# AnjieCheng/SpatialRGPT

Measured on NVIDIA H100. Metric: generated_tokens_per_sec, higher is better.
Workload: dtype bf16

## Files before the change

include/srgpt_b200.h:

```cpp
#ifndef SRGPT_B200_H_
#define SRGPT_B200_H_

#ifdef __cplusplus
extern "C" {
#endif

#define SRGPT_ABI_VERSION 1

int srgpt_abi_version(void);
int srgpt_elem_type(void);
const char* srgpt_last_error(void);
int srgpt_device_info(int* sm_count, int* cc_major, int* cc_minor);

int srgpt_trace_begin(void* device_buf, int capacity_records);
int srgpt_trace_end(void);

enum {
  SRGPT_EPI_NONE = 0,
  SRGPT_EPI_BIAS = 1,
  SRGPT_EPI_BIAS_GELU_TANH = 2,
  SRGPT_EPI_BIAS_GELU_ERF = 3,
  SRGPT_EPI_BIAS_RESIDUAL = 4,
  SRGPT_EPI_SWIGLU = 5,
  SRGPT_EPI_BIAS_QUICK_GELU = 6
};
long long srgpt_gemm_workspace_bytes(void);
int srgpt_gemm_set_workspace(void* workspace, long long bytes);
int srgpt_gemm_bf16(const void* A, int lda, const void* W, int ldw, void* C, int ldc, int M, int N, int K,
                    const void* bias , const void* residual , int ldr,
                    int res_row_mod , int epilogue, int out_fp32, void* stream);

int srgpt_layernorm_bf16(const void* x, int ldx, const void* weight, const void* bias, void* y, int ldy, int rows,
                         int cols, float eps, int act, void* stream);
int srgpt_downsample_layernorm_bf16(const void* x, const void* weight, const void* bias, void* y, int n_img, int side,
                                    int C, float eps, void* stream);
int srgpt_rmsnorm_bf16(const void* x, int ldx, const void* weight, void* y, int ldy, int rows, int cols, float eps,
                       void* stream);
int srgpt_patchify_bf16(const void* images, int src_is_bf16, void* A, int n, int R, int ps, int ldk, void* stream);
int srgpt_clip_embed_bf16(const void* patch_embeds, const void* class_embedding, const void* position_embedding, void* out,
                          int n_img, int T, int D, void* stream);
int srgpt_splice_rows_bf16(const void* src0, const void* src1, const void* src2, const void* src3, const int* src_id,
                           const int* src_row, void* out, int rows, int cols, void* stream);

long long srgpt_mask_weights_workspace(int n_img, int M, int side);
int srgpt_mask_weights(const void* masks, int mask_is_bf16, void* w, void* workspace, int n_img, int M, int IH, int IW,
                       int side, float rscale, int order, void* stream);
long long srgpt_mask_pool_workspace(int n_img, int M, int L, int C);
int srgpt_mask_pool_bf16(const void* x, const void* w, void* out, void* workspace, int n_img, int M, int L, int C,
                         void* stream);
int srgpt_adaptive_avgpool_bf16(const void* x, void* y, int n_img, int side, int out_side, int C, int order,
                                void* stream);
int srgpt_reorder_rows_bf16(const void* x, void* y, int n_img, int side, int C, int from_order, int to_order,
                            void* stream);
int srgpt_depth_to_u8x3(const void* depth, int h, int w, void* out, int H, int W, void* workspace, void* stream);

int srgpt_attention_prefill_bf16(const void* q, const void* k, const void* v, void* out, int q_ld, int kv_ld, int o_ld,
                                 int batch, int seqlen, int n_heads, int n_kv_heads, int head_dim, float scale,
                                 int causal, void* stream);
int srgpt_attention_prefill_varlen_bf16(const void* q, const void* k, const void* v, void* out, int q_ld, int kv_ld,
                                        int o_ld, int n_seqs, const int* cu_seqlens, int max_seqlen, int total_rows,
                                        int n_heads, int n_kv_heads, int head_dim, float scale, int causal, void* stream);
int srgpt_rope_kv_append_bf16(void* qkv, int rows, int n_heads, int n_kv_heads, int head_dim, const void* cos_tab,
                              const void* sin_tab, const int* start_pos, void* kv_pages, const int* page_table,
                              int page_size, void* stream);
int srgpt_rope_kv_append_varlen_bf16(void* qkv, int rows, int n_heads, int n_kv_heads, int head_dim, const void* cos_tab,
                                     const void* sin_tab, const int* start_pos, void* kv_pages, const int* page_tables,
                                     int page_table_stride, int page_size, int n_seqs, const int* cu_seqlens, void* stream);
int srgpt_attention_prefill_paged_bf16(const void* q, int q_ld, void* out, int o_ld, const void* kv_pages, int n_pages,
                                       const int* page_tables, int page_table_stride, int page_size, const int* start_pos,
                                       const int* cu_seqlens, int n_seqs, int max_rows, int total_rows, int n_heads, int n_kv_heads,
                                       int head_dim, float scale, void* stream);
int srgpt_rows_equal(const void* a, const void* b, int rows, long long row_bytes, int* flags, void* stream);
int srgpt_attention_decode_bf16(const void* q, void* out, const void* kv_pages, const int* page_table, int page_size,
                                const int* kv_len_minus1, int n_heads, int n_kv_heads, int head_dim, float scale,
                                void* stream);

enum { SRGPT_GEMV_PLAIN = 0, SRGPT_GEMV_SWIGLU = 1, SRGPT_GEMV_QKV_ROPE = 2 };
int srgpt_gemv_bf16(const void* x, const void* W, int ldw, void* y, int N, int K, const void* norm_weight, float eps,
                    const void* residual, int mode,
                     int n_heads, int n_kv_heads, int head_dim, const void* cos_tab,
                    const void* sin_tab, const int* pos, void* kv_pages, const int* page_table, int page_size,
                    void* stream);
long long srgpt_lm_head_workspace(int V);
// ... 273 lines not shown
```

spatialrgpt_b200/_lib.py:

```python
from __future__ import annotations

import ctypes as C
import os
import threading

from . import _build

_lock = threading.Lock()
_libs = {}
_elem = "bf16"


class SrgptError(RuntimeError):
    pass


vp, ci, cf, cll = C.c_void_p, C.c_int, C.c_float, C.c_longlong

SIGNATURES = {
    "srgpt_abi_version": (ci, []),
    "srgpt_elem_type": (ci, []),
    "srgpt_last_error": (C.c_char_p, []),
    "srgpt_device_info": (ci, [C.POINTER(ci), C.POINTER(ci), C.POINTER(ci)]),
    "srgpt_trace_begin": (ci, [vp, ci]),
    "srgpt_trace_end": (ci, []),
    "srgpt_gemm_workspace_bytes": (cll, []),
    "srgpt_gemm_set_workspace": (ci, [vp, cll]),
    "srgpt_gemm_bf16": (ci, [vp, ci, vp, ci, vp, ci, ci, ci, ci, vp, vp, ci, ci, ci, ci, vp]),
    "srgpt_layernorm_bf16": (ci, [vp, ci, vp, vp, vp, ci, ci, ci, cf, ci, vp]),
    "srgpt_downsample_layernorm_bf16": (ci, [vp, vp, vp, vp, ci, ci, ci, cf, vp]),
    "srgpt_rmsnorm_bf16": (ci, [vp, ci, vp, vp, ci, ci, ci, cf, vp]),
    "srgpt_patchify_bf16": (ci, [vp, ci, vp, ci, ci, ci, ci, vp]),
    "srgpt_clip_embed_bf16": (ci, [vp, vp, vp, vp, ci, ci, ci, vp]),
    "srgpt_splice_rows_bf16": (ci, [vp, vp, vp, vp, vp, vp, vp, ci, ci, vp]),
    "srgpt_mask_weights_workspace": (cll, [ci, ci, ci]),
    "srgpt_mask_weights": (ci, [vp, ci, vp, vp, ci, ci, ci, ci, ci, cf, ci, vp]),
    "srgpt_mask_pool_workspace": (cll, [ci, ci, ci, ci]),
    "srgpt_mask_pool_bf16": (ci, [vp, vp, vp, vp, ci, ci, ci, ci, vp]),
    "srgpt_adaptive_avgpool_bf16": (ci, [vp, vp, ci, ci, ci, ci, ci, vp]),
    "srgpt_reorder_rows_bf16": (ci, [vp, vp, ci, ci, ci, ci, ci, vp]),
    "srgpt_depth_to_u8x3": (ci, [vp, ci, ci, vp, ci, ci, vp, vp]),
    "srgpt_attention_prefill_bf16": (ci, [vp, vp, vp, vp, ci, ci, ci, ci, ci, ci, ci, ci, cf, ci, vp]),
    "srgpt_attention_prefill_varlen_bf16": (ci, [vp, vp, vp, vp, ci, ci, ci, ci, vp, ci, ci, ci, ci, ci, cf, ci, vp]),
    "srgpt_rope_kv_append_bf16": (ci, [vp, ci, ci, ci, ci, vp, vp, vp, vp, vp, ci, vp]),
    "srgpt_rope_kv_append_varlen_bf16": (ci, [vp, ci, ci, ci, ci, vp, vp, vp, vp, vp, ci, ci, ci, vp, vp]),
    "srgpt_attention_prefill_paged_bf16": (ci, [vp, ci, vp, ci, vp, ci, vp, ci, ci, vp, vp, ci, ci, ci, ci, ci, ci, cf, vp]),
    "srgpt_rows_equal": (ci, [vp, vp, ci, cll, vp, vp]),
    "srgpt_attention_decode_bf16": (ci, [vp, vp, vp, vp, ci, vp, ci, ci, ci, cf, vp]),
    "srgpt_gemv_bf16": (ci, [vp, vp, ci, vp, ci, ci, vp, cf, vp, ci, ci, ci, ci, vp, vp, vp, vp, vp, ci, vp]),
    "srgpt_lm_head_workspace": (cll, [ci]),
    "srgpt_lm_head_argmax_bf16": (ci, [vp, vp, ci, ci, ci, vp, cf, vp, vp, vp, vp, vp, vp, vp, vp]),
    "srgpt_argmax_f32": (ci, [vp, ci, ci, vp, vp]),
    "srgpt_argmax_bf16": (ci, [vp, ci, ci, ci, vp, vp]),
    "srgpt_beam_candidates_bf16": (ci, [vp, ci, ci, ci, vp, ci, vp, vp, vp]),
    "srgpt_beam_candidates_scores_bf16": (ci, [vp, ci, ci, ci, vp, ci, vp, vp, vp, cll, vp]),
    "srgpt_step_scores": (ci, [vp, ci, cll, ci, ci, vp, ci, vp, cll, cll, vp]),
    "srgpt_beam_select": (ci, [vp, vp, ci, ci, ci, vp, vp, vp, vp]),
    "srgpt_kv_copy_workspace_bytes": (cll, [ci, ci, ci, ci]),
    "srgpt_kv_copy_pages": (ci, [vp, ci, ci, ci, ci, vp, ci, ci, vp, cll, vp]),
    "srgpt_token_logprobs": (ci, [vp, cll, ci, ci, vp, vp, ci, vp, cll, vp, vp, vp, vp]),
    "srgpt_sample_top_p_f32": (ci, [vp, ci, vp, vp, vp, ci, vp, vp, vp, ci, vp]),
    "srgpt_sample_rows": (ci, [vp, ci, ci, ci, ci, vp, vp, vp, ci, vp, vp]),
    "srgpt_sample_top_p_scores_f32": (ci, [vp, ci, vp, vp, vp, ci, vp, vp, vp, ci, vp, cll, vp]),
    "srgpt_sample_rows_scores": (ci, [vp, ci, ci, ci, ci, vp, vp, vp, ci, vp, vp, cll, vp]),
    "srgpt_logits_process": (ci, [vp, ci, ci, ci, ci, vp, ci, ci, ci, vp, ci, vp, vp, ci, vp, ci, vp, vp]),
    "srgpt_logits_pick_token": (ci, [vp, vp, ci, vp, vp, vp, ci, vp]),
    "srgpt_resample_u8": (ci, [vp, vp, ci, ci, ci, ci, ci, vp, vp, ci, vp]),
    "srgpt_u8_to_normalized_chw": (ci, [vp, vp, ci, ci, ci, C.c_double, vp, vp, ci, vp]),
    "srgpt_resize_nearest_u8": (ci, [vp, vp, ci, ci, ci, ci, vp, vp, vp]),
    "srgpt_attention_decode_batched_bf16": (ci, [vp, ci, vp, ci, vp, vp, ci, ci, vp, ci, ci, ci, ci, cf, vp]),
    "srgpt_decode_batch_advance": (ci, [vp, vp, vp, ci, vp, vp, vp, ci, vp, vp]),
    "srgpt_gemv_tp_bf16": (ci, [vp, vp, ci, vp, ci, ci, vp, cf, ci, ci, ci, ci, vp, vp, vp, vp, vp, ci, ci, ci, vp, vp]),
    "srgpt_attention_decode_tp_bf16": (ci, [vp, vp, vp, vp, ci, vp, ci, ci, ci, ci, ci, cf, vp]),
    "srgpt_tp_residual_add_bf16": (ci, [vp, vp, ci, vp]),
    "srgpt_lm_head_local_best_bf16": (ci, [vp, vp, ci, ci, ci, vp, cf, vp, ci, vp, vp]),
    "srgpt_tp_pick_token": (ci, [vp, ci, vp, vp, ci, vp, vp, vp, vp]),
    "srgpt_tp_comm_bytes": (cll, [ci, ci, ci]),
    "srgpt_tp_comm_slot_offset": (cll, [ci, ci, ci]),
    "srgpt_tp_allreduce_residual_bf16": (ci, [vp, ci, ci, cll, ci, vp, vp, vp, ci, vp]),
    "srgpt_tp_allgather_pick_token": (ci, [vp, ci, ci, cll, ci, vp, vp, vp, ci, vp, vp, vp, vp]),
    "srgpt_siglip_layers_bf16": (ci, [vp, vp, ci, vp, vp, vp, vp, ci, ci, ci, ci, ci, cf, vp]),
# ... 169 lines not shown
```

spatialrgpt_b200/csrc/gemm_wgmma.cu:

```cuda
#include <cuda.h>
#include <stdlib.h>

#include "common.cuh"
#include "nf4.cuh"
#include "srgpt_b200.h"
#include "tma.cuh"

namespace srgpt {
namespace gemm {

using namespace tma;

constexpr int BM = 128, BN = 128, BK = 64;
constexpr int WG_K = 16;
constexpr int STAGES = 6;
constexpr int A_BYTES = BM * BK * 2;
constexpr int B_BYTES = BN * BK * 2;
constexpr int STAGE_BYTES = A_BYTES + B_BYTES;
constexpr int NUM_THREADS = 3 * 128;
constexpr int SMEM_BYTES = STAGES * STAGE_BYTES + 1024  + 256 ;
constexpr int TSK_MAX_CTAS = 256;
constexpr int TSK_FLAG_BYTES = TSK_MAX_CTAS * 4;
constexpr long long TSK_SLOT_FLOATS = (long long)BM * BN;

__device__ __forceinline__ unsigned int ld_acquire_u32(const unsigned int* p) {
  unsigned int v;
  asm volatile("ld.acquire.gpu.global.u32 %0, [%1];" : "=r"(v) : "l"(p) : "memory");
  return v;
}
__device__ __forceinline__ void st_release_u32(unsigned int* p, unsigned int v) {
  asm volatile("st.release.gpu.global.u32 [%0], %1;" ::"l"(p), "r"(v) : "memory");
}

__device__ __forceinline__ void wgmma_m64n128k16(float (&d)[64], uint64_t desc_a, uint64_t desc_b) {
  asm volatile(
      "{\n\t.reg .pred p;\n\tsetp.ne.b32 p, 1, 0;\n\t"
      "wgmma.mma_async.sync.aligned.m64n128k16.f32." SRGPT_ELEM_PTX "." SRGPT_ELEM_PTX " "
      "{%0, %1, %2, %3, %4, %5, %6, %7, %8, %9, %10, %11, %12, %13, %14, %15, "
      "%16, %17, %18, %19, %20, %21, %22, %23, %24, %25, %26, %27, %28, %29, %30, %31, "
      "%32, %33, %34, %35, %36, %37, %38, %39, %40, %41, %42, %43, %44, %45, %46, %47, "
      "%48, %49, %50, %51, %52, %53, %54, %55, %56, %57, %58, %59, %60, %61, %62, %63}, "
      "%64, %65, p, 1, 1, 0, 0;\n\t}"
      : "+f"(d[0]), "+f"(d[1]), "+f"(d[2]), "+f"(d[3]), "+f"(d[4]), "+f"(d[5]), "+f"(d[6]), "+f"(d[7]),
        "+f"(d[8]), "+f"(d[9]), "+f"(d[10]), "+f"(d[11]), "+f"(d[12]), "+f"(d[13]), "+f"(d[14]), "+f"(d[15]),
        "+f"(d[16]), "+f"(d[17]), "+f"(d[18]), "+f"(d[19]), "+f"(d[20]), "+f"(d[21]), "+f"(d[22]), "+f"(d[23]),
        "+f"(d[24]), "+f"(d[25]), "+f"(d[26]), "+f"(d[27]), "+f"(d[28]), "+f"(d[29]), "+f"(d[30]), "+f"(d[31]),
        "+f"(d[32]), "+f"(d[33]), "+f"(d[34]), "+f"(d[35]), "+f"(d[36]), "+f"(d[37]), "+f"(d[38]), "+f"(d[39]),
        "+f"(d[40]), "+f"(d[41]), "+f"(d[42]), "+f"(d[43]), "+f"(d[44]), "+f"(d[45]), "+f"(d[46]), "+f"(d[47]),
        "+f"(d[48]), "+f"(d[49]), "+f"(d[50]), "+f"(d[51]), "+f"(d[52]), "+f"(d[53]), "+f"(d[54]), "+f"(d[55]),
        "+f"(d[56]), "+f"(d[57]), "+f"(d[58]), "+f"(d[59]), "+f"(d[60]), "+f"(d[61]), "+f"(d[62]), "+f"(d[63])
      : "l"(desc_a), "l"(desc_b)
      : "memory");
}

__device__ __forceinline__ void wgmma_m64n128k32_e4m3(float (&d)[64], uint64_t desc_a, uint64_t desc_b) {
  asm volatile(
      "{\n\t.reg .pred p;\n\tsetp.ne.b32 p, 1, 0;\n\t"
      "wgmma.mma_async.sync.aligned.m64n128k32.f32.e4m3.e4m3 "
      "{%0, %1, %2, %3, %4, %5, %6, %7, %8, %9, %10, %11, %12, %13, %14, %15, "
      "%16, %17, %18, %19, %20, %21, %22, %23, %24, %25, %26, %27, %28, %29, %30, %31, "
      "%32, %33, %34, %35, %36, %37, %38, %39, %40, %41, %42, %43, %44, %45, %46, %47, "
      "%48, %49, %50, %51, %52, %53, %54, %55, %56, %57, %58, %59, %60, %61, %62, %63}, "
      "%64, %65, p, 1, 1;\n\t}"
      : "+f"(d[0]), "+f"(d[1]), "+f"(d[2]), "+f"(d[3]), "+f"(d[4]), "+f"(d[5]), "+f"(d[6]), "+f"(d[7]),
        "+f"(d[8]), "+f"(d[9]), "+f"(d[10]), "+f"(d[11]), "+f"(d[12]), "+f"(d[13]), "+f"(d[14]), "+f"(d[15]),
        "+f"(d[16]), "+f"(d[17]), "+f"(d[18]), "+f"(d[19]), "+f"(d[20]), "+f"(d[21]), "+f"(d[22]), "+f"(d[23]),
        "+f"(d[24]), "+f"(d[25]), "+f"(d[26]), "+f"(d[27]), "+f"(d[28]), "+f"(d[29]), "+f"(d[30]), "+f"(d[31]),
        "+f"(d[32]), "+f"(d[33]), "+f"(d[34]), "+f"(d[35]), "+f"(d[36]), "+f"(d[37]), "+f"(d[38]), "+f"(d[39]),
        "+f"(d[40]), "+f"(d[41]), "+f"(d[42]), "+f"(d[43]), "+f"(d[44]), "+f"(d[45]), "+f"(d[46]), "+f"(d[47]),
        "+f"(d[48]), "+f"(d[49]), "+f"(d[50]), "+f"(d[51]), "+f"(d[52]), "+f"(d[53]), "+f"(d[54]), "+f"(d[55]),
        "+f"(d[56]), "+f"(d[57]), "+f"(d[58]), "+f"(d[59]), "+f"(d[60]), "+f"(d[61]), "+f"(d[62]), "+f"(d[63])
      : "l"(desc_a), "l"(desc_b)
      : "memory");
}

struct Fp8Scales {
  const float* sx;
  const float* sw;
};

struct Params {
  int M, N, K;
  int ldc;
  const bf16* bias;
  const bf16* residual;
  int ldr;
  int res_row_mod;
  void* C;
  int out_fp32;
  int gm;
};

struct TskWs {
  float* partial;
  unsigned int* flags;
  unsigned int epoch;
};

__device__ __forceinline__ void unit_to_tile(int unit, int tiles_m, int tiles_n, int gm, int& mt, int& nt) {
  const int per_group = gm * tiles_n;
  const int g = unit / per_group;
  const int rem = unit - g * per_group;
  const int g0 = g * gm;
  const int gsz = min(gm, tiles_m - g0);
  nt = rem / gsz;
  mt = g0 + rem - nt * gsz;
}

template <int EPI>
__device__ __forceinline__ void store_acc(const float (&d)[64], const Params& p, int row0, int col0) {
#pragma unroll
  for (int i = 0; i < 2; ++i) {
    const int row = row0 + 8 * i;
    if (row >= p.M) continue;
    const int rrow = p.res_row_mod > 0 ? row % p.res_row_mod : row;
#pragma unroll
    for (int j = 0; j < 16; ++j) {
      const int col = col0 + 8 * j;
      if (col >= p.N) continue;
      const bool two = col + 1 < p.N;
      float v0 = d[4 * j + 2 * i], v1 = d[4 * j + 2 * i + 1];
      if (EPI == SRGPT_EPI_SWIGLU) {
        const float g = bf16_round(v0), u = bf16_round(v1);
        reinterpret_cast<bf16*>(p.C)[(size_t)row * p.ldc + (col >> 1)] = f2e(bf16_round(silu(g)) * u);
        continue;
      }
      if (EPI != SRGPT_EPI_NONE && p.bias != nullptr) {
        if (two) {
          const uint32_t b = *reinterpret_cast<const uint32_t*>(p.bias + col);
          v0 += bf16_lo(b);
          v1 += bf16_hi(b);
        } else {
          v0 += e2f(p.bias[col]);
        }
      }
      if (EPI == SRGPT_EPI_BIAS_GELU_TANH) {
        v0 = gelu_tanh(bf16_round(v0)); v1 = gelu_tanh(bf16_round(v1));
      } else if (EPI == SRGPT_EPI_BIAS_GELU_ERF) {
        v0 = gelu_erf(bf16_round(v0)); v1 = gelu_erf(bf16_round(v1));
      } else if (EPI == SRGPT_EPI_BIAS_QUICK_GELU) {
        v0 = quick_gelu(bf16_round(v0)); v1 = quick_gelu(bf16_round(v1));
      } else if (EPI == SRGPT_EPI_BIAS_RESIDUAL && p.residual != nullptr) {
        const bf16* rp = p.residual + (size_t)rrow * p.ldr + col;
        if (two) {
          const uint32_t r = *reinterpret_cast<const uint32_t*>(rp);
          v0 = bf16_round(v0) + bf16_lo(r);
          v1 = bf16_round(v1) + bf16_hi(r);
        } else {
          v0 = bf16_round(v0) + e2f(rp[0]);
        }
      }
      if (p.out_fp32) {
        float* cp = reinterpret_cast<float*>(p.C) + (size_t)row * p.ldc + col;
        if (two && (p.ldc & 1) == 0) {
          *reinterpret_cast<float2*>(cp) = make_float2(v0, v1);
        } else {
          cp[0] = v0;
          if (two) cp[1] = v1;
        }
      } else {
        bf16* cp = reinterpret_cast<bf16*>(p.C) + (size_t)row * p.ldc + col;
        if (two) {
          *reinterpret_cast<uint32_t*>(cp) = pack_bf16x2(v0, v1);
        } else {
          cp[0] = f2e(v0);
        }
      }
    }
  }
}
// ... 4 lines not shown
    const int row = row0 + 8 * i;
    if (row >= p.M) continue;
    const float sx = sc.sx[row];
#pragma unroll
    for (int j = 0; j < 16; ++j) {
      const int col = col0 + 8 * j;
#pragma unroll
      for (int c = 0; c < 2; ++c)
        if (col + c < p.N) d[4 * j + 2 * i + c] *= sx * sc.sw[col + c];
    }
  }
}

__device__ __forceinline__ void fence_proxy_async_shared() { asm volatile("fence.proxy.async.shared::cta;" ::: "memory"); }

struct Nf4Raw {
  uint32_t w[8];
  float s[8];
};

__device__ __forceinline__ void nf4_coords(bool sk, int i, int u_begin, int num_kb, int cta, int G, int tiles_m, int tiles_n, int gm, int& m0,
                                           int& n0, int& kb) {
  if (sk) {
    const int u = u_begin + i, tile = u / num_kb;
    m0 = 0;
    n0 = tile * BN;
    kb = u - tile * num_kb;
  } else {
    const int ui = i / num_kb;
    int mt, nt;
    unit_to_tile(cta + ui * G, tiles_m, tiles_n, gm, mt, nt);
    m0 = mt * BM;
    n0 = nt * BN;
    kb = i - ui * num_kb;
  }
}

__device__ __forceinline__ void nf4_fetch(const srgpt_nf4& w4, const Params& p, int n0, int kb, int r0, int j, Nf4Raw& c) {
  const size_t row_bytes = (size_t)(p.K >> 1);
  const int row_scales = p.K / nf4::BLOCK;
  const uint8_t* q = w4.q + (size_t)(n0 + r0) * row_bytes + nf4::lane_offset(8 * kb + j);
  const float* s = w4.scale + (size_t)(n0 + r0) * row_scales + kb;
#pragma unroll
  for (int i = 0; i < 8; ++i) {
    c.w[i] = 0x77777777u;
    c.s[i] = 0.f;
    if (n0 + r0 + 16 * i < p.N) {
      c.w[i] = __ldg(reinterpret_cast<const uint32_t*>(q + (size_t)(16 * i) * row_bytes));
      c.s[i] = __ldg(s + (size_t)(16 * i) * row_scales);
    }
  }
}

template <int EPI, bool SK, bool FP8, bool NF4 = false>
__device__ __forceinline__ void gemm_body(const CUtensorMap* tmap_a, const CUtensorMap* tmap_b, const Params& p, const TskWs& ws, const Fp8Scales& sc,
                                          const srgpt_nf4& w4 = srgpt_nf4{nullptr, nullptr}) {
  constexpr int KB = FP8 ? 128 : BK;
  extern __shared__ uint8_t smem_raw[];
  uint8_t* smem = reinterpret_cast<uint8_t*>((reinterpret_cast<uintptr_t>(smem_raw) + 1023) & ~(uintptr_t)1023);
  uint64_t* full_bar = reinterpret_cast<uint64_t*>(smem + STAGES * STAGE_BYTES);
  uint64_t* empty_bar = full_bar + STAGES;

  const int tiles_m = (p.M + BM - 1) / BM;
  const int tiles_n = (p.N + BN - 1) / BN;
  const int num_kb = (p.K + KB - 1) / KB;
  const int num_units = tiles_m * tiles_n;
  const int G = (int)gridDim.x, cta = (int)blockIdx.x;
  const long long total = (long long)tiles_n * num_kb;
  auto range_begin = [&](int c) { return (int)(total * c / G); };
  const int u_begin = SK ? range_begin(cta) : 0, u_end = SK ? range_begin(cta + 1) : 0;

  float* nf4_tab = reinterpret_cast<float*>(empty_bar + STAGES);
  if constexpr (NF4) {
    if (threadIdx.x < 16) nf4_tab[threadIdx.x] = nf4::code_value(threadIdx.x);
  }
  if (threadIdx.x == 0) {
    prefetch_tmap(tmap_a);
    if constexpr (!NF4) prefetch_tmap(tmap_b);
    for (int s = 0; s < STAGES; ++s) {
      mbar_init(smem_u32(&full_bar[s]), NF4 ? 1 + 128 : 1);
      mbar_init(smem_u32(&empty_bar[s]), 2);
    }
    fence_barrier_init();
  }
  __syncthreads();

  const int wg = threadIdx.x >> 7;
  if constexpr (NF4) {
    if (wg == 0) {
      const int pt = threadIdx.x, j = pt & 7, r0 = pt >> 3;
      const int n_loads = SK ? u_end - u_begin : (cta < num_units ? (num_units - 1 - cta) / G + 1 : 0) * num_kb;
      uint32_t stage = 0, phase = 0;
      auto fetch = [&](int i, Nf4Raw& c) {
        int m0, n0, kb;
        nf4_coords(SK, i, u_begin, num_kb, cta, G, tiles_m, tiles_n, p.gm, m0, n0, kb);
        nf4_fetch(w4, p, n0, kb, r0, j, c);
      };
      auto put = [&](int i, const Nf4Raw& c) {
        int m0, n0, kb;
        nf4_coords(SK, i, u_begin, num_kb, cta, G, tiles_m, tiles_n, p.gm, m0, n0, kb);
        mbar_wait(smem_u32(&empty_bar[stage]), phase ^ 1);
        const uint32_t fb = smem_u32(&full_bar[stage]);
        uint8_t* sa = smem + stage * STAGE_BYTES;
        if (pt == 0) {
          mbar_expect_tx(fb, A_BYTES);
          tma_load_2d(smem_u32(sa), tmap_a, fb, kb * BK, m0);
        }
        uint8_t* sb = sa + A_BYTES + r0 * 128 + ((j ^ (r0 & 7)) << 4);
#pragma unroll
        for (int i2 = 0; i2 < 8; ++i2) *reinterpret_cast<uint4*>(sb + i2 * 16 * 128) = nf4::dequant8(c.w[i2], c.s[i2], nf4_tab);
        fence_proxy_async_shared();
        mbar_arrive(fb);
        if (++stage == STAGES) { stage = 0; phase ^= 1; }
      };
      Nf4Raw b0, b1, b2;
      if (n_loads > 0) fetch(0, b0);
      if (n_loads > 1) fetch(1, b1);
      if (n_loads > 2) fetch(2, b2);
      for (int i = 0; i < n_loads; i += 3) {
        put(i, b0);
        if (i + 3 < n_loads) fetch(i + 3, b0);
        if (i + 1 < n_loads) {
          put(i + 1, b1);
          if (i + 4 < n_loads) fetch(i + 4, b1);
        }
        if (i + 2 < n_loads) {
          put(i + 2, b2);
          if (i + 5 < n_loads) fetch(i + 5, b2);
        }
      }
      return;
    }
  }
  if (wg == 0) {
    if (threadIdx.x == 0) {
      uint32_t stage = 0, phase = 0;
      auto load = [&](int m0, int n0, int kb) {
        mbar_wait(smem_u32(&empty_bar[stage]), phase ^ 1);
        const uint32_t fb = smem_u32(&full_bar[stage]);
        mbar_expect_tx(fb, STAGE_BYTES);
        uint8_t* sa = smem + stage * STAGE_BYTES;
        tma_load_2d(smem_u32(sa), tmap_a, fb, kb * KB, m0);
        tma_load_2d(smem_u32(sa + A_BYTES), tmap_b, fb, kb * KB, n0);
        if (++stage == STAGES) { stage = 0; phase ^= 1; }
      };
      if (SK) {
        for (int u = u_begin; u < u_end; ++u) {
          const int tile = u / num_kb;
          load(0, tile * BN, u - tile * num_kb);
        }
      } else {
        for (int unit = cta; unit < num_units; unit += G) {
          int mt, nt;
          unit_to_tile(unit, tiles_m, tiles_n, p.gm, mt, nt);
          for (int kb = 0; kb < num_kb; ++kb) load(mt * BM, nt * BN, kb);
        }
      }
    }
    return;
  }

  const int t = threadIdx.x & 127, ct = threadIdx.x - 128;
  const int r_in_tile = (wg - 1) * 64 + ((t >> 5) << 4) + ((t & 31) >> 2);
  const int c_in_tile = (t & 3) * 2;
  uint32_t stage = 0, phase = 0;
  float d[64];
  auto mainloop = [&](int n) {
#pragma unroll
    for (int i = 0; i < 64; ++i) d[i] = 0.f;
    uint32_t prev = 0;
    for (int kb = 0; kb < n; ++kb) {
      mbar_wait(smem_u32(&full_bar[stage]), phase);
      const uint32_t a_addr = smem_u32(smem + stage * STAGE_BYTES) + (wg - 1) * 64 * 128;
      const uint32_t b_addr = smem_u32(smem + stage * STAGE_BYTES + A_BYTES);
      const uint64_t a_desc = make_desc_sw128(a_addr), b_desc = make_desc_sw128(b_addr);
      wgmma_fence();
#pragma unroll
      for (int k = 0; k < BK / WG_K; ++k) {
        if constexpr (FP8)
          wgmma_m64n128k32_e4m3(d, a_desc + (uint64_t)(2 * k), b_desc + (uint64_t)(2 * k));
        else
          wgmma_m64n128k16(d, a_desc + (uint64_t)(2 * k), b_desc + (uint64_t)(2 * k));
      }
      wgmma_commit();
      if (kb > 0) {
        wgmma_wait<1>();
        if (t == 0) mbar_arrive(smem_u32(&empty_bar[prev]));
      }
      prev = stage;
      if (++stage == STAGES) { stage = 0; phase ^= 1; }
    }
    wgmma_wait<0>();
    if (t == 0 && n > 0) mbar_arrive(smem_u32(&empty_bar[prev]));
  };

  if (!SK) {
    for (int unit = cta; unit < num_units; unit += G) {
      int mt, nt;
      unit_to_tile(unit, tiles_m, tiles_n, p.gm, mt, nt);
      mainloop(num_kb);
      if constexpr (FP8) scale_acc(d, sc, p, mt * BM + r_in_tile, nt * BN + c_in_tile);
      store_acc<EPI>(d, p, mt * BM + r_in_tile, nt * BN + c_in_tile);
    }
    return;
  }

  int u = u_begin;
  while (u < u_end) {
    const int tile = u / num_kb;
    const int seg_end = min(u_end, (tile + 1) * num_kb);
    const bool owner = u == tile * num_kb;
    int c_last = cta;
    if (owner && seg_end < (tile + 1) * num_kb) {
      const int last_unit = (tile + 1) * num_kb - 1;
      while (c_last + 1 < G && range_begin(c_last + 1) <= last_unit) ++c_last;
    }
    mainloop(seg_end - u);
    float* slot = ws.partial + (size_t)cta * (BM * BN);
    if (!owner) {
#pragma unroll
      for (int i = 0; i < 64; ++i) __stcg(slot + i * 256 + ct, d[i]);
      __threadfence();
      named_bar_sync(1, 256);
      if (ct == 0) st_release_u32(ws.flags + cta, ws.epoch);
    } else {
      for (int cc = cta + 1; cc <= c_last; ++cc) {
        if ((t & 31) == 0) {
          uint32_t spins = 0;
          while (ld_acquire_u32(ws.flags + cc) != ws.epoch) {
            __nanosleep(64);
            if (++spins > (1u << 24)) __trap();
          }
        }
        __syncwarp();
        const float* src = ws.partial + (size_t)cc * (BM * BN);
#pragma unroll
        for (int i = 0; i < 64; ++i) d[i] += __ldcg(src + i * 256 + ct);
      }
      if constexpr (FP8) scale_acc(d, sc, p, r_in_tile, tile * BN + c_in_tile);
      store_acc<EPI>(d, p, r_in_tile, tile * BN + c_in_tile);
      if (c_last > cta) {
        named_bar_sync(1, 256);
        if (ct == 0)
          for (int cc = cta + 1; cc <= c_last; ++cc) st_release_u32(ws.flags + cc, 0u);
      }
    }
    u = seg_end;
  }
}

template <int EPI, bool SK>
__global__ void __launch_bounds__(NUM_THREADS, 1)
gemm_kernel(const __grid_constant__ CUtensorMap tmap_a, const __grid_constant__ CUtensorMap tmap_b, const Params p, const TskWs ws) {
  gemm_body<EPI, SK, false>(&tmap_a, &tmap_b, p, ws, Fp8Scales{nullptr, nullptr});
}

template <int EPI, bool SK>
__global__ void __launch_bounds__(NUM_THREADS, 1)
gemm_fp8_kernel(const __grid_constant__ CUtensorMap tmap_a, const __grid_constant__ CUtensorMap tmap_b, const Params p, const TskWs ws,
                const Fp8Scales sc) {
  gemm_body<EPI, SK, true>(&tmap_a, &tmap_b, p, ws, sc);
}

template <int EPI, bool SK>
__global__ void __launch_bounds__(NUM_THREADS, 1)
gemm_nf4_kernel(const __grid_constant__ CUtensorMap tmap_a, const Params p, const TskWs ws, const srgpt_nf4 w4) {
  gemm_body<EPI, SK, false, true>(&tmap_a, nullptr, p, ws, Fp8Scales{nullptr, nullptr}, w4);
}

static int make_tmap(CUtensorMap* tm, const void* ptr, int rows, int k, int ld, bool fp8 = false) {
  const cuuint64_t dims[2] = {(cuuint64_t)k, (cuuint64_t)rows};
  const cuuint64_t strides[1] = {(cuuint64_t)ld * (fp8 ? 1 : 2)};
  const cuuint32_t box[2] = {fp8 ? 128u : (cuuint32_t)BK, 128u};
  const int r = fp8 ? encode_tmap(tm, CU_TENSOR_MAP_DATA_TYPE_UINT8, ptr, 2, dims, strides, box, CU_TENSOR_MAP_SWIZZLE_128B)
                    : encode_tmap_bf16(tm, ptr, 2, dims, strides, box, CU_TENSOR_MAP_SWIZZLE_128B);
  if (r != 0) {
    set_last_error("cuTensorMapEncodeTiled failed: %d (rows=%d k=%d ld=%d ptr=%p)", r, rows, k, ld, ptr);
    return SRGPT_ERR_CUDA;
  }
  return SRGPT_OK;
}

static int env_int(const char* name) {
  const char* v = getenv(name);
  return (v != nullptr && v[0] != 0) ? atoi(v) : 0;
}

struct TskState {
  void* base = nullptr;
  long long bytes = 0;
  unsigned int epoch = 0;
};
static TskState g_tsk;

static long long tsk_workspace_bytes(int ctas) { return TSK_FLAG_BYTES + (long long)ctas * TSK_SLOT_FLOATS * 4; }

template <int EPI, bool SK, bool FP8, bool NF4>
static int launch_kernel(const CUtensorMap& ta, const CUtensorMap& tb, const Params& p, const TskWs& ws, const Fp8Scales& sc, const srgpt_nf4& w4,
                         int grid, cudaStream_t stream) {
  static bool configured = false;
  if (!configured) {
    if constexpr (NF4)
      SRGPT_CHECK_CUDA(cudaFuncSetAttribute(gemm_nf4_kernel<EPI, SK>, cudaFuncAttributeMaxDynamicSharedMemorySize, SMEM_BYTES));
    else if constexpr (FP8)
      SRGPT_CHECK_CUDA(cudaFuncSetAttribute(gemm_fp8_kernel<EPI, SK>, cudaFuncAttributeMaxDynamicSharedMemorySize, SMEM_BYTES));
    else
      SRGPT_CHECK_CUDA(cudaFuncSetAttribute(gemm_kernel<EPI, SK>, cudaFuncAttributeMaxDynamicSharedMemorySize, SMEM_BYTES));
    configured = true;
  }
  if constexpr (NF4)
    gemm_nf4_kernel<EPI, SK><<<grid, NUM_THREADS, SMEM_BYTES, stream>>>(ta, p, ws, w4);
  else if constexpr (FP8)
    gemm_fp8_kernel<EPI, SK><<<grid, NUM_THREADS, SMEM_BYTES, stream>>>(ta, tb, p, ws, sc);
  else
    gemm_kernel<EPI, SK><<<grid, NUM_THREADS, SMEM_BYTES, stream>>>(ta, tb, p, ws);
  SRGPT_CHECK_LAUNCH();
  return SRGPT_OK;
}

template <int EPI, bool FP8 = false, bool NF4 = false>
static int launch(const void* A, int lda, const void* W, int ldw, const Params& p, cudaStream_t stream, const Fp8Scales& sc = Fp8Scales{nullptr, nullptr},
                  const srgpt_nf4& w4 = srgpt_nf4{nullptr, nullptr}) {
  constexpr int EB = FP8 ? 1 : 2;
  constexpr int KB = FP8 ? 128 : BK;
  CUtensorMap ta, tb;
  int rc = make_tmap(&ta, A, p.M, p.K, lda, FP8);
  if (rc != SRGPT_OK) return rc;
  if (!NF4) {
    rc = make_tmap(&tb, W, p.N, p.K, ldw, FP8);
    if (rc != SRGPT_OK) return rc;
  }
  const int sms = sm_count();
  TskWs ws = {nullptr, nullptr, 0};
  static const int tsk_env = env_int("SRGPT_GEMM_TSK");
  const long long sk_units = (long long)ceil_div(p.N, BN) * ceil_div(p.K, KB);
  if (tsk_env >= 0 && g_tsk.base != nullptr && p.M <= BM && (long long)p.N * p.K * EB >= (4LL << 20) &&
      g_tsk.bytes >= tsk_workspace_bytes(8)) {
    int grid = sms < TSK_MAX_CTAS ? sms : TSK_MAX_CTAS;
    if ((long long)grid > sk_units) grid = (int)sk_units;
    while (tsk_workspace_bytes(grid) > g_tsk.bytes && grid > 1) --grid;
    ws.flags = reinterpret_cast<unsigned int*>(g_tsk.base);
    ws.partial = reinterpret_cast<float*>(reinterpret_cast<uint8_t*>(g_tsk.base) + TSK_FLAG_BYTES);
    if (++g_tsk.epoch == 0) g_tsk.epoch = 1;
    ws.epoch = g_tsk.epoch;
    return launch_kernel<EPI, true, FP8, NF4>(ta, tb, p, ws, sc, w4, grid, stream);
  }
  static const int gm_env = env_int("SRGPT_GEMM_GM");
  const int tiles_m = ceil_div(p.M, BM);
  Params pg = p;
  pg.gm = tiles_m;
  if ((double)EB * p.M * p.K > 40e6) {
    const int g = (int)(20e6 / ((double)EB * BM * p.K));
    pg.gm = g < 1 ? 1 : (g < tiles_m ? g : tiles_m);
  }
  if (gm_env > 0) pg.gm = gm_env < tiles_m ? gm_env : tiles_m;
  const long long units = (long long)tiles_m * ceil_div(p.N, BN);
  const int grid = (int)(units < sms ? units : sms);
  return launch_kernel<EPI, false, FP8, NF4>(ta, tb, pg, ws, sc, w4, grid, stream);
}

}
}

using namespace srgpt;

extern "C" __attribute__((visibility("default"))) long long srgpt_gemm_workspace_bytes(void) {
  int n = sm_count();
  if (n <= 0 || n > gemm::TSK_MAX_CTAS) n = gemm::TSK_MAX_CTAS;
  return gemm::tsk_workspace_bytes(n);
}

extern "C" __attribute__((visibility("default"))) int srgpt_gemm_set_workspace(void* workspace, long long bytes) {
  if (workspace == nullptr || bytes <= 0) {
    gemm::g_tsk = gemm::TskState{};
    return SRGPT_OK;
  }
  SRGPT_CHECK_ARG((reinterpret_cast<uintptr_t>(workspace) & 1023) == 0 && bytes >= gemm::tsk_workspace_bytes(8));
  gemm::g_tsk.base = workspace;
  gemm::g_tsk.bytes = bytes;
  gemm::g_tsk.epoch = 0;
  return SRGPT_OK;
}

extern "C" __attribute__((visibility("default"))) int srgpt_gemm_bf16(const void* A, int lda, const void* W, int ldw, void* C, int ldc, int M, int N, int K,
                               const void* bias, const void* residual, int ldr, int res_row_mod, int epilogue,
                               int out_fp32, void* stream) {
  SRGPT_CHECK_ARG(A != nullptr && W != nullptr && C != nullptr);
  SRGPT_CHECK_ARG(M > 0 && N > 0 && K > 0);
  SRGPT_CHECK_ARG(lda >= K && ldw >= K);
  SRGPT_CHECK_ARG((lda % 8) == 0 && (ldw % 8) == 0);
  SRGPT_CHECK_ARG((reinterpret_cast<uintptr_t>(A) & 15) == 0 && (reinterpret_cast<uintptr_t>(W) & 15) == 0);
  SRGPT_CHECK_ARG((reinterpret_cast<uintptr_t>(C) & 15) == 0);
  SRGPT_CHECK_ARG(epilogue >= SRGPT_EPI_NONE && epilogue <= SRGPT_EPI_BIAS_QUICK_GELU);
  if (epilogue == SRGPT_EPI_SWIGLU) {
    SRGPT_CHECK_ARG((N % 2) == 0 && !out_fp32 && ldc >= N / 2 && (ldc % 8) == 0);
  } else {
    SRGPT_CHECK_ARG(ldc >= N);
    SRGPT_CHECK_ARG(out_fp32 || (ldc % 8) == 0);
  }
  if (residual != nullptr) {
    SRGPT_CHECK_ARG(epilogue == SRGPT_EPI_BIAS_RESIDUAL && ldr >= N && (ldr % 8) == 0);
    SRGPT_CHECK_ARG((reinterpret_cast<uintptr_t>(residual) & 15) == 0);
  }
  if (bias != nullptr) SRGPT_CHECK_ARG((reinterpret_cast<uintptr_t>(bias) & 15) == 0);

  gemm::Params p;
  p.gm = 1;
  p.M = M; p.N = N; p.K = K; p.ldc = ldc;
  p.bias = reinterpret_cast<const bf16*>(bias);
  p.residual = reinterpret_cast<const bf16*>(residual);
  p.ldr = ldr; p.res_row_mod = res_row_mod;
  p.C = C; p.out_fp32 = out_fp32;

  cudaStream_t st = reinterpret_cast<cudaStream_t>(stream);
  switch (epilogue) {
    case SRGPT_EPI_NONE: return gemm::launch<SRGPT_EPI_NONE>(A, lda, W, ldw, p, st);
    case SRGPT_EPI_BIAS: return gemm::launch<SRGPT_EPI_BIAS>(A, lda, W, ldw, p, st);
    case SRGPT_EPI_BIAS_GELU_TANH: return gemm::launch<SRGPT_EPI_BIAS_GELU_TANH>(A, lda, W, ldw, p, st);
    case SRGPT_EPI_BIAS_GELU_ERF: return gemm::launch<SRGPT_EPI_BIAS_GELU_ERF>(A, lda, W, ldw, p, st);
    case SRGPT_EPI_BIAS_RESIDUAL: return gemm::launch<SRGPT_EPI_BIAS_RESIDUAL>(A, lda, W, ldw, p, st);
    case SRGPT_EPI_SWIGLU: return gemm::launch<SRGPT_EPI_SWIGLU>(A, lda, W, ldw, p, st);
    case SRGPT_EPI_BIAS_QUICK_GELU: return gemm::launch<SRGPT_EPI_BIAS_QUICK_GELU>(A, lda, W, ldw, p, st);
  }
  return SRGPT_ERR_INVALID;
}

extern "C" __attribute__((visibility("default"))) int srgpt_gemm_fp8_bf16(const void* A, int lda, const float* sx, const void* W, int ldw, const float* sw,
                                                                            void* C, int ldc, int M, int N, int K, const void* residual, int ldr,
                                                                            int epilogue, void* stream) {
  SRGPT_CHECK_ARG(A != nullptr && W != nullptr && C != nullptr && sx != nullptr && sw != nullptr);
  SRGPT_CHECK_ARG(M > 0 && N > 0 && K > 0 && (K % 16) == 0);
  SRGPT_CHECK_ARG(lda >= K && ldw >= K && (lda % 16) == 0 && (ldw % 16) == 0);
  SRGPT_CHECK_ARG((reinterpret_cast<uintptr_t>(A) & 15) == 0 && (reinterpret_cast<uintptr_t>(W) & 15) == 0);
// ... 66 lines not shown
```

Before: 225.4.

## Add 128x256 wgmma tile path for large bf16 GEMMs with shared planner

```diff
diff --git a/include/srgpt_b200.h b/include/srgpt_b200.h
--- a/include/srgpt_b200.h
+++ b/include/srgpt_b200.h
@@ -29,6 +29,10 @@
 int srgpt_gemm_bf16(const void* A, int lda, const void* W, int ldw, void* C, int ldc, int M, int N, int K,
                     const void* bias , const void* residual , int ldr,
                     int res_row_mod , int epilogue, int out_fp32, void* stream);
+typedef struct {
+  int stream_k, tile_m, tile_n, group_m, grid;
+} srgpt_gemm_plan_t;
+int srgpt_gemm_plan(int M, int N, int K, int elem_bytes, int sms, int workspace, srgpt_gemm_plan_t* out);
 
 int srgpt_layernorm_bf16(const void* x, int ldx, const void* weight, const void* bias, void* y, int ldy, int rows,
                          int cols, float eps, int act, void* stream);
diff --git a/spatialrgpt_b200/_lib.py b/spatialrgpt_b200/_lib.py
--- a/spatialrgpt_b200/_lib.py
+++ b/spatialrgpt_b200/_lib.py
@@ -27,6 +27,7 @@
     "srgpt_gemm_workspace_bytes": (cll, []),
     "srgpt_gemm_set_workspace": (ci, [vp, cll]),
     "srgpt_gemm_bf16": (ci, [vp, ci, vp, ci, vp, ci, ci, ci, ci, vp, vp, ci, ci, ci, ci, vp]),
+    "srgpt_gemm_plan": (ci, [ci, ci, ci, ci, ci, ci, vp]),
     "srgpt_layernorm_bf16": (ci, [vp, ci, vp, vp, vp, ci, ci, ci, cf, ci, vp]),
     "srgpt_downsample_layernorm_bf16": (ci, [vp, vp, vp, vp, ci, ci, ci, cf, vp]),
     "srgpt_rmsnorm_bf16": (ci, [vp, ci, vp, vp, ci, ci, ci, cf, vp]),
diff --git a/spatialrgpt_b200/csrc/gemm_wgmma.cu b/spatialrgpt_b200/csrc/gemm_wgmma.cu
--- a/spatialrgpt_b200/csrc/gemm_wgmma.cu
+++ b/spatialrgpt_b200/csrc/gemm_wgmma.cu
@@ -22,6 +22,15 @@
 constexpr int TSK_MAX_CTAS = 256;
 constexpr int TSK_FLAG_BYTES = TSK_MAX_CTAS * 4;
 constexpr long long TSK_SLOT_FLOATS = (long long)BM * BN;
+constexpr int MAX_SMEM = 227 * 1024;
+
+template <int TN>
+struct Ring {
+  static constexpr int STAGE_BYTES = A_BYTES + TN * BK * 2;
+  static constexpr int STAGES = (MAX_SMEM - 1280) / STAGE_BYTES < gemm::STAGES ? (MAX_SMEM - 1280) / STAGE_BYTES : gemm::STAGES;
+  static constexpr int SMEM_BYTES = STAGES * STAGE_BYTES + 1024  + 256 ;
+};
+static_assert(Ring<BN>::STAGES == STAGES && Ring<BN>::SMEM_BYTES == SMEM_BYTES, "Ring<128> is the 128 x 128 ring");
 
 __device__ __forceinline__ unsigned int ld_acquire_u32(const unsigned int* p) {
   unsigned int v;
@@ -53,6 +62,40 @@
       : "memory");
 }
 
+template <int TN>
+__device__ __forceinline__ void wgmma_ss(float (&d)[TN / 2], uint64_t desc_a, uint64_t desc_b);
+template <>
+__device__ __forceinline__ void wgmma_ss<128>(float (&d)[64], uint64_t desc_a, uint64_t desc_b) {
+  wgmma_m64n128k16(d, desc_a, desc_b);
+}
+
+template <>
+__device__ __forceinline__ void wgmma_ss<256>(float (&d)[128], uint64_t desc_a, uint64_t desc_b) {
+  asm volatile(
+      "{\n\t.reg .pred p;\n\tsetp.ne.b32 p, 1, 0;\n\t"
+      "wgmma.mma_async.sync.aligned.m64n256k16.f32." SRGPT_ELEM_PTX "." SRGPT_ELEM_PTX " "
+      "{%0, %1, %2, %3, %4, %5, %6, %7, %8, %9, %10, %11, %12, %13, %14, %15, %16, %17, %18, %19, %20, %21, %22, %23, %24, %25, %26, %27, %28, %29, %30, %31, %32, %33, %34, %35, %36, %37, %38, %39, %40, %41, %42, %43, %44, %45, %46, %47, %48, %49, %50, %51, %52, %53, %54, %55, %56, %57, %58, %59, %60, %61, %62, %63, %64, %65, %66, %67, %68, %69, %70, %71, %72, %73, %74, %75, %76, %77, %78, %79, %80, %81, %82, %83, %84, %85, %86, %87, %88, %89, %90, %91, %92, %93, %94, %95, %96, %97, %98, %99, %100, %101, %102, %103, %104, %105, %106, %107, %108, %109, %110, %111, %112, %113, %114, %115, %116, %117, %118, %119, %120, %121, %122, %123, %124, %125, %126, %127}, "
+      "%128, %129, p, 1, 1, 0, 0;\n\t}"
+      : "+f"(d[0]), "+f"(d[1]), "+f"(d[2]), "+f"(d[3]), "+f"(d[4]), "+f"(d[5]), "+f"(d[6]), "+f"(d[7]),
+        "+f"(d[8]), "+f"(d[9]), "+f"(d[10]), "+f"(d[11]), "+f"(d[12]), "+f"(d[13]), "+f"(d[14]), "+f"(d[15]),
+        "+f"(d[16]), "+f"(d[17]), "+f"(d[18]), "+f"(d[19]), "+f"(d[20]), "+f"(d[21]), "+f"(d[22]), "+f"(d[23]),
+        "+f"(d[24]), "+f"(d[25]), "+f"(d[26]), "+f"(d[27]), "+f"(d[28]), "+f"(d[29]), "+f"(d[30]), "+f"(d[31]),
+        "+f"(d[32]), "+f"(d[33]), "+f"(d[34]), "+f"(d[35]), "+f"(d[36]), "+f"(d[37]), "+f"(d[38]), "+f"(d[39]),
+        "+f"(d[40]), "+f"(d[41]), "+f"(d[42]), "+f"(d[43]), "+f"(d[44]), "+f"(d[45]), "+f"(d[46]), "+f"(d[47]),
+        "+f"(d[48]), "+f"(d[49]), "+f"(d[50]), "+f"(d[51]), "+f"(d[52]), "+f"(d[53]), "+f"(d[54]), "+f"(d[55]),
+        "+f"(d[56]), "+f"(d[57]), "+f"(d[58]), "+f"(d[59]), "+f"(d[60]), "+f"(d[61]), "+f"(d[62]), "+f"(d[63]),
+        "+f"(d[64]), "+f"(d[65]), "+f"(d[66]), "+f"(d[67]), "+f"(d[68]), "+f"(d[69]), "+f"(d[70]), "+f"(d[71]),
+        "+f"(d[72]), "+f"(d[73]), "+f"(d[74]), "+f"(d[75]), "+f"(d[76]), "+f"(d[77]), "+f"(d[78]), "+f"(d[79]),
+        "+f"(d[80]), "+f"(d[81]), "+f"(d[82]), "+f"(d[83]), "+f"(d[84]), "+f"(d[85]), "+f"(d[86]), "+f"(d[87]),
+        "+f"(d[88]), "+f"(d[89]), "+f"(d[90]), "+f"(d[91]), "+f"(d[92]), "+f"(d[93]), "+f"(d[94]), "+f"(d[95]),
+        "+f"(d[96]), "+f"(d[97]), "+f"(d[98]), "+f"(d[99]), "+f"(d[100]), "+f"(d[101]), "+f"(d[102]), "+f"(d[103]),
+        "+f"(d[104]), "+f"(d[105]), "+f"(d[106]), "+f"(d[107]), "+f"(d[108]), "+f"(d[109]), "+f"(d[110]), "+f"(d[111]),
+        "+f"(d[112]), "+f"(d[113]), "+f"(d[114]), "+f"(d[115]), "+f"(d[116]), "+f"(d[117]), "+f"(d[118]), "+f"(d[119]),
+        "+f"(d[120]), "+f"(d[121]), "+f"(d[122]), "+f"(d[123]), "+f"(d[124]), "+f"(d[125]), "+f"(d[126]), "+f"(d[127])
+      : "l"(desc_a), "l"(desc_b)
+      : "memory");
+}
+
 __device__ __forceinline__ void wgmma_m64n128k32_e4m3(float (&d)[64], uint64_t desc_a, uint64_t desc_b) {
   asm volatile(
       "{\n\t.reg .pred p;\n\tsetp.ne.b32 p, 1, 0;\n\t"
@@ -107,15 +150,15 @@
   mt = g0 + rem - nt * gsz;
 }
 
-template <int EPI>
-__device__ __forceinline__ void store_acc(const float (&d)[64], const Params& p, int row0, int col0) {
+template <int EPI, int J = 16>
+__device__ __forceinline__ void store_acc(const float (&d)[4 * J], const Params& p, int row0, int col0) {
 #pragma unroll
   for (int i = 0; i < 2; ++i) {
     const int row = row0 + 8 * i;
     if (row >= p.M) continue;
     const int rrow = p.res_row_mod > 0 ? row % p.res_row_mod : row;
 #pragma unroll
-    for (int j = 0; j < 16; ++j) {
+    for (int j = 0; j < J; ++j) {
       const int col = col0 + 8 * j;
       if (col >= p.N) continue;
       const bool two = col + 1 < p.N;
@@ -226,17 +269,19 @@
   }
 }
 
-template <int EPI, bool SK, bool FP8, bool NF4 = false>
+template <int EPI, bool SK, bool FP8, bool NF4 = false, int TN = BN>
 __device__ __forceinline__ void gemm_body(const CUtensorMap* tmap_a, const CUtensorMap* tmap_b, const Params& p, const TskWs& ws, const Fp8Scales& sc,
                                           const srgpt_nf4& w4 = srgpt_nf4{nullptr, nullptr}) {
   constexpr int KB = FP8 ? 128 : BK;
+  constexpr int STAGES = Ring<TN>::STAGES, STAGE_BYTES = Ring<TN>::STAGE_BYTES;
+  static_assert(TN == BN || !(SK || FP8 || NF4), "stream-K, FP8 and NF4 run the 128 x 128 tile only");
   extern __shared__ uint8_t smem_raw[];
   uint8_t* smem = reinterpret_cast<uint8_t*>((reinterpret_cast<uintptr_t>(smem_raw) + 1023) & ~(uintptr_t)1023);
   uint64_t* full_bar = reinterpret_cast<uint64_t*>(smem + STAGES * STAGE_BYTES);
   uint64_t* empty_bar = full_bar + STAGES;
 
   const int tiles_m = (p.M + BM - 1) / BM;
-  const int tiles_n = (p.N + BN - 1) / BN;
+  const int tiles_n = (p.N + TN - 1) / TN;
   const int num_kb = (p.K + KB - 1) / KB;
   const int num_units = tiles_m * tiles_n;
   const int G = (int)gridDim.x, cta = (int)blockIdx.x;
@@ -327,7 +372,7 @@
         for (int unit = cta; unit < num_units; unit += G) {
           int mt, nt;
           unit_to_tile(unit, tiles_m, tiles_n, p.gm, mt, nt);
-          for (int kb = 0; kb < num_kb; ++kb) load(mt * BM, nt * BN, kb);
+          for (int kb = 0; kb < num_kb; ++kb) load(mt * BM, nt * TN, kb);
         }
       }
     }
@@ -338,10 +383,10 @@
   const int r_in_tile = (wg - 1) * 64 + ((t >> 5) << 4) + ((t & 31) >> 2);
   const int c_in_tile = (t & 3) * 2;
   uint32_t stage = 0, phase = 0;
-  float d[64];
+  float d[TN / 2];
   auto mainloop = [&](int n) {
 #pragma unroll
-    for (int i = 0; i < 64; ++i) d[i] = 0.f;
+    for (int i = 0; i < TN / 2; ++i) d[i] = 0.f;
     uint32_t prev = 0;
     for (int kb = 0; kb < n; ++kb) {
       mbar_wait(smem_u32(&full_bar[stage]), phase);
@@ -354,7 +399,7 @@
         if constexpr (FP8)
           wgmma_m64n128k32_e4m3(d, a_desc + (uint64_t)(2 * k), b_desc + (uint64_t)(2 * k));
         else
-          wgmma_m64n128k16(d, a_desc + (uint64_t)(2 * k), b_desc + (uint64_t)(2 * k));
+          wgmma_ss<TN>(d, a_desc + (uint64_t)(2 * k), b_desc + (uint64_t)(2 * k));
       }
       wgmma_commit();
       if (kb > 0) {
@@ -373,8 +418,8 @@
       int mt, nt;
       unit_to_tile(unit, tiles_m, tiles_n, p.gm, mt, nt);
       mainloop(num_kb);
-      if constexpr (FP8) scale_acc(d, sc, p, mt * BM + r_in_tile, nt * BN + c_in_tile);
-      store_acc<EPI>(d, p, mt * BM + r_in_tile, nt * BN + c_in_tile);
+      if constexpr (FP8) scale_acc(d, sc, p, mt * BM + r_in_tile, nt * TN + c_in_tile);
+      store_acc<EPI, TN / 8>(d, p, mt * BM + r_in_tile, nt * TN + c_in_tile);
     }
     return;
   }
@@ -412,7 +457,7 @@
         for (int i = 0; i < 64; ++i) d[i] += __ldcg(src + i * 256 + ct);
       }
       if constexpr (FP8) scale_acc(d, sc, p, r_in_tile, tile * BN + c_in_tile);
-      store_acc<EPI>(d, p, r_in_tile, tile * BN + c_in_tile);
+      store_acc<EPI, TN / 8>(d, p, r_in_tile, tile * BN + c_in_tile);
       if (c_last > cta) {
         named_bar_sync(1, 256);
         if (ct == 0)
@@ -423,10 +468,10 @@
   }
 }
 
-template <int EPI, bool SK>
+template <int EPI, bool SK, int TN = BN>
 __global__ void __launch_bounds__(NUM_THREADS, 1)
 gemm_kernel(const __grid_constant__ CUtensorMap tmap_a, const __grid_constant__ CUtensorMap tmap_b, const Params p, const TskWs ws) {
-  gemm_body<EPI, SK, false>(&tmap_a, &tmap_b, p, ws, Fp8Scales{nullptr, nullptr});
+  gemm_body<EPI, SK, false, false, TN>(&tmap_a, &tmap_b, p, ws, Fp8Scales{nullptr, nullptr});
 }
 
 template <int EPI, bool SK>
@@ -442,10 +487,10 @@
   gemm_body<EPI, SK, false, true>(&tmap_a, nullptr, p, ws, Fp8Scales{nullptr, nullptr}, w4);
 }
 
-static int make_tmap(CUtensorMap* tm, const void* ptr, int rows, int k, int ld, bool fp8 = false) {
+static int make_tmap(CUtensorMap* tm, const void* ptr, int rows, int k, int ld, bool fp8 = false, int box_rows = 128) {
   const cuuint64_t dims[2] = {(cuuint64_t)k, (cuuint64_t)rows};
   const cuuint64_t strides[1] = {(cuuint64_t)ld * (fp8 ? 1 : 2)};
-  const cuuint32_t box[2] = {fp8 ? 128u : (cuuint32_t)BK, 128u};
+  const cuuint32_t box[2] = {fp8 ? 128u : (cuuint32_t)BK, (cuuint32_t)box_rows};
   const int r = fp8 ? encode_tmap(tm, CU_TENSOR_MAP_DATA_TYPE_UINT8, ptr, 2, dims, strides, box, CU_TENSOR_MAP_SWIZZLE_128B)
                     : encode_tmap_bf16(tm, ptr, 2, dims, strides, box, CU_TENSOR_MAP_SWIZZLE_128B);
   if (r != 0) {
@@ -469,7 +514,7 @@
 
 static long long tsk_workspace_bytes(int ctas) { return TSK_FLAG_BYTES + (long long)ctas * TSK_SLOT_FLOATS * 4; }
 
-template <int EPI, bool SK, bool FP8, bool NF4>
+template <int EPI, bool SK, bool FP8, bool NF4, int TN = BN>
 static int launch_kernel(const CUtensorMap& ta, const CUtensorMap& tb, const Params& p, const TskWs& ws, const Fp8Scales& sc, const srgpt_nf4& w4,
                          int grid, cudaStream_t stream) {
   static bool configured = false;
@@ -479,7 +524,7 @@
     else if constexpr (FP8)
       SRGPT_CHECK_CUDA(cudaFuncSetAttribute(gemm_fp8_kernel<EPI, SK>, cudaFuncAttributeMaxDynamicSharedMemorySize, SMEM_BYTES));
     else
-      SRGPT_CHECK_CUDA(cudaFuncSetAttribute(gemm_kernel<EPI, SK>, cudaFuncAttributeMaxDynamicSharedMemorySize, SMEM_BYTES));
+      SRGPT_CHECK_CUDA(cudaFuncSetAttribute(gemm_kernel<EPI, SK, TN>, cudaFuncAttributeMaxDynamicSharedMemorySize, Ring<TN>::SMEM_BYTES));
     configured = true;
   }
   if constexpr (NF4)
@@ -487,31 +532,75 @@
   else if constexpr (FP8)
     gemm_fp8_kernel<EPI, SK><<<grid, NUM_THREADS, SMEM_BYTES, stream>>>(ta, tb, p, ws, sc);
   else
-    gemm_kernel<EPI, SK><<<grid, NUM_THREADS, SMEM_BYTES, stream>>>(ta, tb, p, ws);
+    gemm_kernel<EPI, SK, TN><<<grid, NUM_THREADS, Ring<TN>::SMEM_BYTES, stream>>>(ta, tb, p, ws);
   SRGPT_CHECK_LAUNCH();
   return SRGPT_OK;
+}
+
+struct Plan {
+  int stream_k;
+  int tn;
+  int gm;
+  int grid;
+};
+
+static bool wide_tile_pays(int M, int N, int K, int sms) {
+  return K >= 2048 && (long long)ceil_div(M, BM) * ceil_div(N, BN) >= 4LL * sms;
+}
+
+static Plan make_plan(int M, int N, int K, int elem_bytes, int sms, bool workspace, int mode, int tsk_env, int gm_env) {
+  const int kb = elem_bytes == 1 ? 128 : BK;
+  Plan pl = {0, BN, 1, 1};
+  if (tsk_env >= 0 && workspace && M <= BM && (long long)N * K * elem_bytes >= (4LL << 20)) {
+    const long long sk_units = (long long)ceil_div(N, BN) * ceil_div(K, kb);
+    pl.stream_k = 1;
+    pl.grid = sms < TSK_MAX_CTAS ? sms : TSK_MAX_CTAS;
+    if ((long long)pl.grid > sk_units) pl.grid = (int)sk_units;
+    return pl;
+  }
+  if (elem_bytes == 2 && mode != 0 && wide_tile_pays(M, N, K, sms)) pl.tn = 256;
+  const int tiles_m = ceil_div(M, BM);
+  pl.gm = tiles_m;
+  if ((double)elem_bytes * M * K > 40e6) {
+    const int g = (int)(20e6 / ((double)elem_bytes * BM * K));
+    pl.gm = g < 1 ? 1 : (g < tiles_m ? g : tiles_m);
+  }
+  if (gm_env > 0) pl.gm = gm_env < tiles_m ? gm_env : tiles_m;
+  const long long units = (long long)tiles_m * ceil_div(N, pl.tn);
+  pl.grid = (int)(units < sms ? units : sms);
+  return pl;
+}
+
+static int plan_mode() {
+  static const int mode = [] {
+    const char* v = getenv("SRGPT_GEMM_PLAN");
+    return (v != nullptr && v[0] != 0 && atoi(v) == 0) ? 0 : 1;
+  }();
+  return mode;
+}
+
+static Plan plan_for(int M, int N, int K, int elem_bytes, int mode, int sms, bool workspace) {
+  static const int tsk_env = env_int("SRGPT_GEMM_TSK");
+  static const int gm_env = env_int("SRGPT_GEMM_GM");
+  return make_plan(M, N, K, elem_bytes, sms, workspace, mode, tsk_env, gm_env);
 }
 
 template <int EPI, bool FP8 = false, bool NF4 = false>
 static int launch(const void* A, int lda, const void* W, int ldw, const Params& p, cudaStream_t stream, const Fp8Scales& sc = Fp8Scales{nullptr, nullptr},
                   const srgpt_nf4& w4 = srgpt_nf4{nullptr, nullptr}) {
   constexpr int EB = FP8 ? 1 : 2;
-  constexpr int KB = FP8 ? 128 : BK;
+  const Plan pl = plan_for(p.M, p.N, p.K, EB, FP8 || NF4 ? 0 : plan_mode(), sm_count(),
+                           g_tsk.base != nullptr && g_tsk.bytes >= tsk_workspace_bytes(8));
   CUtensorMap ta, tb;
   int rc = make_tmap(&ta, A, p.M, p.K, lda, FP8);
   if (rc != SRGPT_OK) return rc;
   if (!NF4) {
-    rc = make_tmap(&tb, W, p.N, p.K, ldw, FP8);
+    rc = make_tmap(&tb, W, p.N, p.K, ldw, FP8, pl.tn);
     if (rc != SRGPT_OK) return rc;
   }
-  const int sms = sm_count();
   TskWs ws = {nullptr, nullptr, 0};
-  static const int tsk_env = env_int("SRGPT_GEMM_TSK");
-  const long long sk_units = (long long)ceil_div(p.N, BN) * ceil_div(p.K, KB);
-  if (tsk_env >= 0 && g_tsk.base != nullptr && p.M <= BM && (long long)p.N * p.K * EB >= (4LL << 20) &&
-      g_tsk.bytes >= tsk_workspace_bytes(8)) {
-    int grid = sms < TSK_MAX_CTAS ? sms : TSK_MAX_CTAS;
-    if ((long long)grid > sk_units) grid = (int)sk_units;
+  if (pl.stream_k) {
+    int grid = pl.grid;
     while (tsk_workspace_bytes(grid) > g_tsk.bytes && grid > 1) --grid;
     ws.flags = reinterpret_cast<unsigned int*>(g_tsk.base);
     ws.partial = reinterpret_cast<float*>(reinterpret_cast<uint8_t*>(g_tsk.base) + TSK_FLAG_BYTES);
@@ -519,18 +608,12 @@
     ws.epoch = g_tsk.epoch;
     return launch_kernel<EPI, true, FP8, NF4>(ta, tb, p, ws, sc, w4, grid, stream);
   }
-  static const int gm_env = env_int("SRGPT_GEMM_GM");
-  const int tiles_m = ceil_div(p.M, BM);
   Params pg = p;
-  pg.gm = tiles_m;
-  if ((double)EB * p.M * p.K > 40e6) {
-    const int g = (int)(20e6 / ((double)EB * BM * p.K));
-    pg.gm = g < 1 ? 1 : (g < tiles_m ? g : tiles_m);
-  }
-  if (gm_env > 0) pg.gm = gm_env < tiles_m ? gm_env : tiles_m;
-  const long long units = (long long)tiles_m * ceil_div(p.N, BN);
-  const int grid = (int)(units < sms ? units : sms);
-  return launch_kernel<EPI, false, FP8, NF4>(ta, tb, pg, ws, sc, w4, grid, stream);
+  pg.gm = pl.gm;
+  if constexpr (!FP8 && !NF4) {
+    if (pl.tn == 256) return launch_kernel<EPI, false, false, false, 256>(ta, tb, pg, ws, sc, w4, pl.grid, stream);
+  }
+  return launch_kernel<EPI, false, FP8, NF4>(ta, tb, pg, ws, sc, w4, pl.grid, stream);
 }
 
 }
@@ -553,6 +636,18 @@
   gemm::g_tsk.base = workspace;
   gemm::g_tsk.bytes = bytes;
   gemm::g_tsk.epoch = 0;
+  return SRGPT_OK;
+}
+
+extern "C" __attribute__((visibility("default"))) int srgpt_gemm_plan(int M, int N, int K, int elem_bytes, int sms, int workspace,
+                                                                        srgpt_gemm_plan_t* out) {
+  SRGPT_CHECK_ARG(out != nullptr && M > 0 && N > 0 && K > 0 && sms > 0 && (elem_bytes == 1 || elem_bytes == 2));
+  const gemm::Plan pl = gemm::plan_for(M, N, K, elem_bytes, gemm::plan_mode(), sms, workspace != 0);
+  out->stream_k = pl.stream_k;
+  out->tile_m = gemm::BM;
+  out->tile_n = pl.tn;
+  out->group_m = pl.gm;
+  out->grid = pl.grid;
   return SRGPT_OK;
 }
 
```

Result: no change. 225.5, median of 6 (+0.0%).
